# tensorlayer/HyperPose

Hardware: AMD Instinct MI355X
Metric: end-to-end FPS (preproc+DNN+PAF parse) @ 368x432 (higher is better)
Workload: dtype f32; 1 GPU; configs[1]: Lightweight-OpenPose (MobilenetDilated) + PAF parser, batch 8 @ 368x432 per GPU; frames from pinned host memory (one H2D per batch), parser on the network's own maps, humans to the host; key=configs[1]/f32, global_batch=8, parallelism=frame-sharded x1, no steady-state collective, pipes_per_gpu=4, parser_input=the network's own heat-maps

## Files before the change

### hyperpose_amd/csrc/conv32_winograd.hip

```cpp
#include "conv_fp32.hpp"

#include "conv32_epilogue.hpp"
#include "conv_device.hpp"

#include <cstdlib>
#include <vector>

namespace hp {

namespace {

typedef float f32x4 __attribute__((ext_vector_type(4)));

constexpr int WCK = 16;
constexpr int HALO_W = 10;
constexpr int RAW_PB = WCK * 4;
constexpr int VP = 24 * 4;

template <int MW, int NC = 2>
struct wino_geom {
    static constexpr int NT = 64 * MW;
    static constexpr int HALO_H = 8 * NC + 2;
    static constexpr int RAW_Q = HALO_H * HALO_W * 4;
    static constexpr int NQ = (RAW_Q + NT - 1) / NT;
    static constexpr int RAW_BYTES = NQ * NT * 16;
    static constexpr int NI = 4 * NC / MW;
    static_assert(NI >= 1, "a transform item per wavefront");
    static constexpr int TMS = MW / 2;
    static constexpr int SLAB_PITCH = rows_geom<TMS>::PITCH, SLAB_BYTES = 64 * NC * SLAB_PITCH * 4;
    static constexpr int VPOS = 16 * NC * VP, VBUF = 16 * VPOS;
    static constexpr int LDS_BYTES = RAW_BYTES + (VBUF > SLAB_BYTES ? VBUF : SLAB_BYTES);
    static constexpr int PVPOS = 16 * NC * 64, PVBUF = 16 * PVPOS;
    static constexpr int PLDS_BYTES = RAW_BYTES + (2 * PVBUF > SLAB_BYTES ? 2 * PVBUF : SLAB_BYTES);
};

__device__ __forceinline__ long tvw_off(const tview32& t, int b, int y, int x)
{
    return ((long)b * t.img + (long)y * t.wp + x) * t.cs + t.coff;
}

}

template <int MW, bool PIPE, int NC = 2>
__global__ __launch_bounds__(64 * MW, MW == 8 ? 1 : NC == 1 ? 3 : 2) void conv32_winograd_kernel(const conv32_params p, int tiles_x, int tiles_y, int vh)
{
    static_assert(!PIPE || MW == 4, "the pipelined form is the four-wavefront one");
    using G = wino_geom<MW, NC>;
    constexpr int NT = G::NT, NQ = G::NQ, SLAB_PITCH = G::SLAB_PITCH, RAW_Q = G::RAW_Q, VPOS = G::VPOS;
    extern __shared__ __attribute__((aligned(16))) unsigned char lds[];
    unsigned char* const raw = lds;
    unsigned char* const vb = lds + G::RAW_BYTES;

    const int tid = threadIdx.x, lane = tid & 63, wave = tid >> 6;
    const int NG = p.Cout_pad / (16 * MW), ntiles = tiles_x * tiles_y * (vh ? 1 : p.B);
    const int Hin = vh ? (p.B - 1) * vh + p.H : p.H;
    const int bj = blockIdx.x >> 3, by = bj % NG;
    int t = (bj / NG) * 8 + (blockIdx.x & 7);
    if (t >= ntiles)
        return;
    const int bx = t;
    const int tx = t % tiles_x;
    t /= tiles_x;
    const int ty = t % tiles_y, b = t / tiles_y;
    const int y0 = ty * (8 * NC), x0 = tx * 8;
    const int MT = p.Cout_pad / 16, mt = by * MW + wave;
    const int nch = p.Cin / WCK;
    int dbg_i = 0;
#define HP_STAMP()                                                     \
    if (p.dbg && bx == 1 && by == 0 && tid == 0)       \
        p.dbg[dbg_i++] = __builtin_amdgcn_s_memtime();
    HP_STAMP();
    if (p.dbg && bx == 1 && by == 0 && tid == 0)
        p.dbg[119] = __builtin_readcyclecounter(), p.dbg[120] = __builtin_amdgcn_s_memrealtime();

    long goff[NQ];
    bool qok[NQ];
#pragma unroll
    for (int i = 0; i < NQ; ++i) {
        const int q = min(tid + i * NT, RAW_Q - 1);
        const int hp = q >> 2, c4 = q & 3;
        const int hy = hp / HALO_W, hx = hp - hy * HALO_W;
        const int y = y0 - 1 + hy, x = x0 - 1 + hx;
        qok[i] = y <= Hin && x <= p.W;
        goff[i] = tvw_off(p.in, b, min(y, Hin), min(x, p.W)) + c4 * 4;
    }
    f32x4 stage[NQ];
    auto gload = [&](int c) {
#pragma unroll
        for (int i = 0; i < NQ; ++i)
            stage[i] = *reinterpret_cast<const f32x4*>(p.in.p + goff[i] + min(c, nch - 1) * WCK);
    };
    auto to_lds = [&]() {
#pragma unroll
        for (int i = 0; i < NQ; ++i)
            *reinterpret_cast<f32x4*>(raw + (tid + i * NT) * 16) = qok[i] ? stage[i] : f32x4{ 0.f, 0.f, 0.f, 0.f };
    };
    auto transform = [&]() {
#pragma unroll
        for (int k = 0; k < G::NI; ++k) {
            const int item = wave + k * MW, i = NC == 2 ? item >> 1 : item;
            const int quad = lane >> 4, tile = (NC == 2 ? (item & 1) * 16 : 0) + (lane & 15);
            const int ra = i == 0 ? 0 : i == 2 ? 2 : 1, rb = i == 0 ? 2 : i == 1 ? 2 : i == 2 ? 1 : 3;
            const float sg = i == 1 ? 1.f : -1.f;
            const unsigned char* const src = raw + ((2 * (tile >> 2)) * HALO_W + 2 * (tile & 3)) * RAW_PB + quad * 16;
            f32x4 T[4];
#pragma unroll
            for (int j = 0; j < 4; ++j) {
                const f32x4 a = *reinterpret_cast<const f32x4*>(src + (ra * HALO_W + j) * RAW_PB);
                const f32x4 bq = *reinterpret_cast<const f32x4*>(src + (rb * HALO_W + j) * RAW_PB);
                T[j] = a + sg * bq;
            }
            constexpr int PS = PIPE ? G::PVPOS : VPOS;
            unsigned char* const dst = PIPE ? vb + (i * 4) * PS + tile * 64 + ((quad ^ ((4 - (tile >> 2)) & 3)) * 16) : vb + (i * 4) * PS + tile * VP + quad * 16;
            *reinterpret_cast<f32x4*>(dst) = T[0] - T[2];
            *reinterpret_cast<f32x4*>(dst + PS) = T[1] + T[2];
            *reinterpret_cast<f32x4*>(dst + 2 * PS) = T[2] - T[1];
            *reinterpret_cast<f32x4*>(dst + 3 * PS) = T[1] - T[3];
        }
    };
    f32x4 ta[4], tb[4];
    auto transform_piece = [&](int pos, int buf) {
        const int k = pos >> 3, ps = pos & 7;
        if (k >= G::NI)
            return;
        const int item = wave + k * MW, i = NC == 2 ? item >> 1 : item;
        const int quad = lane >> 4, tile = (NC == 2 ? (item & 1) * 16 : 0) + (lane & 15);
        const int ra = i == 0 ? 0 : i == 2 ? 2 : 1, rb = i == 0 ? 2 : i == 1 ? 2 : i == 2 ? 1 : 3;
        const unsigned char* const src = raw + ((2 * (tile >> 2)) * HALO_W + 2 * (tile & 3)) * RAW_PB + quad * 16;
        if (ps < 4) {
            ta[ps] = *reinterpret_cast<const f32x4*>(src + (ra * HALO_W + ps) * RAW_PB);
            tb[ps] = *reinterpret_cast<const f32x4*>(src + (rb * HALO_W + ps) * RAW_PB);
        } else {
            if (ps == 4) {
                const float sg = i == 1 ? 1.f : -1.f;
#pragma unroll
                for (int j = 0; j < 4; ++j)
                    ta[j] = ta[j] + sg * tb[j];
            }
            unsigned char* const dst = vb + buf * G::PVBUF + (i * 4 + (ps - 4)) * G::PVPOS + tile * 64 + ((quad ^ ((4 - (tile >> 2)) & 3)) * 16);
            *reinterpret_cast<f32x4*>(dst) = ps == 4 ? ta[0] - ta[2] : ps == 5 ? ta[1] + ta[2] : ps == 6 ? ta[2] - ta[1] : ta[1] - ta[3];
        }
    };

    const long step_stride = (long)MT * 256;
    const float* const wp = p.w_wino + (long)mt * 256 + lane * 4;
    const int nsteps = nch * 16;
    constexpr int RING = PIPE ? 4 : 8, AHEAD = PIPE ? 3 : 6;
    f32x4 fa[RING];
    auto aload = [&](int slot, int s) { fa[slot] = *reinterpret_cast<const f32x4*>(wp + (long)min(s, nsteps - 1) * step_stride); };

    f32x4 acc[16][NC];
#pragma unroll
    for (int i = 0; i < 16; ++i)
#pragma unroll
        for (int nc = 0; nc < NC; ++nc)
            acc[i][nc] = f32x4{ 0.f, 0.f, 0.f, 0.f };

    const int btile = lane & 15, kq = lane >> 4;
    const unsigned char* const vsrc = PIPE ? vb + btile * 64 + ((kq ^ ((4 - (btile >> 2)) & 3)) * 16) : vb + btile * VP + kq * 16;
    constexpr int BPOS = PIPE ? G::PVPOS : VPOS, BNT = PIPE ? 16 * 64 : 16 * VP;

    gload(0);
#pragma unroll
    for (int a = 0; a < AHEAD; ++a)
        aload(a, a);
    if constexpr (PIPE) {
        to_lds();
        gload(1);
        lds_barrier();
        transform();
    }
    int s = 0;
#pragma unroll 1
    for (int c = 0; c < nch; ++c) {
        if constexpr (PIPE)
            lds_barrier();
        to_lds();
        gload(PIPE ? c + 2 : c + 1);
        lds_barrier();
        HP_STAMP();
        if constexpr (!PIPE) {
            transform();
            lds_barrier();
            HP_STAMP();
        }
        const unsigned char* const vcur = vsrc + (PIPE ? (c & 1) * G::PVBUF : 0);
        f32x4 fb[2][NC];
#pragma unroll
        for (int nc = 0; nc < NC; ++nc)
            fb[0][nc] = *reinterpret_cast<const f32x4*>(vcur + nc * BNT);
#pragma unroll
        for (int pos = 0; pos < 16; ++pos) {
            const int cur = pos & 1, npos = pos + 1 < 16 ? pos + 1 : pos;
#pragma unroll
            for (int nc = 0; nc < NC; ++nc)
                fb[cur ^ 1][nc] = *reinterpret_cast<const f32x4*>(vcur + npos * BPOS + nc * BNT);
            aload((pos + AHEAD) % RING, s + AHEAD);
            const int slot = pos % RING;
#pragma unroll
            for (int e = 0; e < 4; ++e)
#pragma unroll
                for (int nc = 0; nc < NC; ++nc)
                    acc[pos][nc] = __builtin_amdgcn_mfma_f32_16x16x4f32(fa[slot][e], fb[cur][nc][e], acc[pos][nc], 0, 0, 0);
            if constexpr (PIPE)
                transform_piece(pos, (c + 1) & 1);
            __builtin_amdgcn_sched_group_barrier(0x008, 1, 0);
            __builtin_amdgcn_sched_group_barrier(0x100, 1, 0);
            if constexpr (NC == 2) {
                __builtin_amdgcn_sched_group_barrier(0x008, 1, 0);
                __builtin_amdgcn_sched_group_barrier(0x100, 1, 0);
            }
            __builtin_amdgcn_sched_group_barrier(0x008, 1, 0);
            __builtin_amdgcn_sched_group_barrier(0x020, 1, 0);
            __builtin_amdgcn_sched_group_barrier(0x008, NC == 2 ? 5 : 2, 0);
            __builtin_amdgcn_sched_barrier(0);
            ++s;
        }
        HP_STAMP();
    }

    lds_barrier();
    HP_STAMP();
    float* const slab = reinterpret_cast<float*>(vb);
#pragma unroll
    for (int nt = 0; nt < NC; ++nt) {
        f32x4 S[2][4];
#pragma unroll
        for (int j = 0; j < 4; ++j) {
            S[0][j] = acc[j][nt] + acc[4 + j][nt] + acc[8 + j][nt];
            S[1][j] = acc[4 + j][nt] - acc[8 + j][nt] - acc[12 + j][nt];
        }
#pragma unroll
        for (int a = 0; a < 2; ++a) {
            const f32x4 y0v = S[a][0] + S[a][1] + S[a][2], y1v = S[a][1] - S[a][2] - S[a][3];
            *reinterpret_cast<f32x4*>(slab + ((a * 2 + 0) * (16 * NC) + nt * 16 + btile) * SLAB_PITCH + wave * 16 + kq * 4) = y0v;
            *reinterpret_cast<f32x4*>(slab + ((a * 2 + 1) * (16 * NC) + nt * 16 + btile) * SLAB_PITCH + wave * 16 + kq * 4) = y1v;
        }
    }
    HP_STAMP();
    lds_barrier();
    HP_STAMP();
    constexpr int RPW = 64 * NC / MW;
    conv32_drain_rows<G::TMS, RPW>(p, slab + wave * RPW * SLAB_PITCH, lane, by * 16 * MW, [&](int r, bool& ok, long& ooff, long& roff) {
        const int rr = wave * RPW + r, ab = rr / (16 * NC), tile = rr % (16 * NC);
        int oy = y0 + 2 * (tile >> 2) + (ab >> 1), ob = b;
        const int ox = x0 + 2 * (tile & 3) + (ab & 1);
        if (vh)
            ob = oy / vh, oy -= ob * vh;
        ok = oy < p.OH && ox < p.OW && ob < p.B;
        const int oyc = min(oy, p.OH - 1), oxc = min(ox, p.OW - 1), obc = min(ob, p.B - 1);
        ooff = tvw_off(p.out, obc, oyc, oxc);
        roff = p.res.p ? tvw_off(p.res, obc, oyc, oxc) : 0;
    });
    HP_STAMP();
#undef HP_STAMP
    if (p.dbg && bx == 1 && by == 0 && tid == 0)
        p.dbg[121] = __builtin_readcyclecounter(), p.dbg[122] = __builtin_amdgcn_s_memrealtime();
}

bool conv32_winograd_ok(const conv32_params& p)
{
    return p.KH == 3 && p.KW == 3 && p.stride == 1 && p.dil == 1 && p.Cin % WCK == 0 && p.Cout_pad % 64 == 0 && p.OH == p.H && p.OW == p.W && p.pad_t == 1
        && p.pad_l == 1 && !p.out_f32 && p.out.p;
}

int conv32_winograd_tile(const conv32_params& p) { return p.w_wino3 ? conv32_winograd3_tile(p) : 35000000 + 3000 + 4; }

double conv32_winograd_flops(const conv32_params& p)
{
    return 2.0 * 16 * (double)p.B * ((p.OH + 1) / 2) * ((p.OW + 1) / 2) * p.Cout * p.Cin;
}

void conv32_winograd_pack(const float* packed, int cout_pad, int cin, float* out)
{
    static const double G[4][3] = { { 1, 0, 0 }, { .5, .5, .5 }, { .5, -.5, .5 }, { 0, 0, 1 } };
    const int nch = cin / WCK, MT = cout_pad / 16;
    std::vector<double> U((size_t)16 * cout_pad * cin);
    for (int m = 0; m < cout_pad; ++m)
        for (int k = 0; k < cin; ++k) {
            double g[3][3], Gg[4][3];
            for (int t = 0; t < 9; ++t)
                g[t / 3][t % 3] = packed[((size_t)t * cout_pad + m) * cin + k];
            for (int i = 0; i < 4; ++i)
                for (int j = 0; j < 3; ++j)
                    Gg[i][j] = G[i][0] * g[0][j] + G[i][1] * g[1][j] + G[i][2] * g[2][j];
            for (int i = 0; i < 4; ++i)
                for (int j = 0; j < 4; ++j)
                    U[((size_t)(i * 4 + j) * cout_pad + m) * cin + k] = Gg[i][0] * G[j][0] + Gg[i][1] * G[j][1] + Gg[i][2] * G[j][2];
        }
    for (int c = 0; c < nch; ++c)
        for (int pos = 0; pos < 16; ++pos)
            for (int mt = 0; mt < MT; ++mt) {
                float* dst = out + (((size_t)c * 16 + pos) * MT + mt) * 256;
                for (int lane = 0; lane < 64; ++lane)
                    for (int e = 0; e < 4; ++e) {
                        const int m = mt * 16 + (lane & 15), k = c * WCK + (lane >> 4) * 4 + e;
                        dst[lane * 4 + e] = (float)U[((size_t)pos * cout_pad + m) * cin + k];
                    }
            }
}

template <int MW, bool PIPE, int NC = 2>
static hipError_t launch_wino_case(const conv32_params& q, dim3 grid, int tiles_x, int tiles_y, int vh, hipStream_t s)
{
    constexpr int lds = PIPE ? wino_geom<MW, NC>::PLDS_BYTES : wino_geom<MW, NC>::LDS_BYTES;
    static bool granted = false;
    if (lds > 64 * 1024 && !granted) {
        const hipError_t e = hipFuncSetAttribute((const void*)conv32_winograd_kernel<MW, PIPE, NC>, hipFuncAttributeMaxDynamicSharedMemorySize, lds);
        if (e != hipSuccess)
            return e;
        granted = true;
    }
    HP_LAUNCH((conv32_winograd_kernel<MW, PIPE, NC>), grid, dim3(64 * MW), lds, s, q, tiles_x, tiles_y, vh);
    return hipGetLastError();
}

static int winograd_nc(const conv32_params& p, const engine_switches& sw, int blocks_nc2)
{
    const int force = sw.wino_nc;
    if (force == 1 || force == 2)
        return force;
    return p.latency && blocks_nc2 <= 512 ? 1 : 2;
}

static int winograd_tall(const conv32_params& p, const engine_switches& sw)
{
    if (!sw.wino_tall)
        return 0;
    if (p.B < 2 || p.in.wp <= 0 || p.in.img % p.in.wp)
        return 0;
    const int vh = p.in.img / p.in.wp;
    return (vh & 1) == 0 && vh >= p.H + 2 ? vh : 0;
}

hipError_t launch_conv32_winograd(const conv32_params& p, const engine_switches& sw, hipStream_t s)
{
    if (!conv32_winograd_ok(p) || !p.w_wino || p.npix <= 0)
        return hipErrorInvalidValue;
    constexpr int mw = 4;
    const int tiles_x = (p.OW + 7) / 8;
    const int nc = winograd_nc(p, sw, tiles_x * ((p.OH + 15) / 16) * p.B * (p.Cout_pad / 64)), bh = 8 * nc;
    int tiles_y = (p.OH + bh - 1) / bh, vh = winograd_tall(p, sw), images = p.B;
    if (vh) {
        const int tall_y = ((p.B - 1) * vh + p.H + bh - 1) / bh;
        if (tall_y < tiles_y * p.B)
            tiles_y = tall_y, images = 1;
        else
            vh = 0;
    }
    const dim3 grid((tiles_x * tiles_y * images + 7) / 8 * 8 * (p.Cout_pad / (16 * mw)));
    if (nc == 1)
        return launch_wino_case<4, true, 1>(p, grid, tiles_x, tiles_y, vh, s);
    return launch_wino_case<4, true>(p, grid, tiles_x, tiles_y, vh, s);
}

hipError_t conv32_winograd_occupancy(const conv32_params&, int* blocks_per_cu)
{
    return hipOccupancyMaxActiveBlocksPerMultiprocessor(blocks_per_cu, conv32_winograd_kernel<4, true>, 256, wino_geom<4>::PLDS_BYTES);
}

}
```

### hyperpose_amd/csrc/engine.cpp

```cpp
#include "conv_fp32.hpp"
#include "conv_i8.hpp"
#include "conv_kernels.hpp"
#include "hp_common.hpp"

#include <algorithm>
#include <cmath>
#include <map>
#include <memory>
#include <string>
#include <cstdio>
#include <cstdlib>
#include <vector>

namespace {

inline int round_up(int a, int b) { return (a + b - 1) / b * b; }

struct tensor_info {
    bool defined = false;
    bool elided = false;
    bool unwritten = false;
    int H = 0, W = 0, C = 0;
    int cs = 0;
    int P = 0;
// ... 1478 lines not shown
}

int hp_engine::pair_heads()
{
    const bool f32 = is_f32();
    if (!switches.no_pair_heads && !f32) {
        for (size_t k = 0; k + 1 < steps.size(); ++k) {
            step &a = steps[k], &b = steps[k + 1];
            if (a.op != OP_MLPHEAD || b.op != OP_MLPHEAD || a.paired)
                continue;
            const auto &x = a.hp_, &y = b.hp_;
            if (x.in.p != y.in.p || x.in.coff != y.in.coff || x.K1 != y.K1 || x.H != y.H || x.W != y.W || x.pw.Cout > 64 || y.pw.Cout > 64)
                continue;
            a.hp2_ = b.hp_, a.paired = true, a.n_layers += b.n_layers;
            a.flops += b.flops, a.bytes += b.bytes;
            steps.erase(steps.begin() + k + 1);
        }
    }
    return HP_OK;
}

int hp_engine::finish(const hp_engine_desc* d)
{
    HP_REQUIRE(!steps.empty() && steps[0].first, HP_ERR_INVALID, "engine: the first layer must be a CONV reading tensor 0");

    HP_HIP_TRY(hipStreamCreateWithFlags(&stream, hipStreamNonBlocking));
    HP_HIP_TRY(hipEventCreate(&ev0));
    HP_HIP_TRY(hipEventCreate(&ev1));
    HP_HIP_TRY(hipEventCreateWithFlags(&ev_fork, hipEventDisableTiming));
    HP_HIP_TRY(hipEventCreateWithFlags(&ev_join, hipEventDisableTiming));
    if (dtype == HP_DTYPE_I8) {
        i8_scale.assign(layers.size(), 0.f);
        for (size_t i = 0; i < layers.size(); ++i)
            if (i8_eligible((int)i))
                i8_scale[i] = -1.f;
        if (d->int8_scales) {
            HP_TRY(check_int8_scales(d->int8_scales, d->n_layers, true));
            i8_scale.assign(d->int8_scales, d->int8_scales + d->n_layers);
            for (auto& v : i8_scale)
                v = v < 0.f ? -1.f : v;
        }
        HP_TRY(apply_int8_scales());
    }
    return HP_OK;
}


int hp_engine::check_int8_scales(const float* s, int n, bool allow_uncalibrated) const
{
    HP_REQUIRE(s, HP_ERR_INVALID, "int8 scales: null vector");
    HP_REQUIRE(n == (int)layers.size(), HP_ERR_INVALID, "int8 scales: %d values for %zu layers", n, layers.size());
    for (int i = 0; i < n; ++i) {
        HP_REQUIRE(std::isfinite(s[i]), HP_ERR_INVALID, "int8 scales: layer %d: %g is not finite", i, (double)s[i]);
        const bool uncal = allow_uncalibrated && s[i] == -1.f && i8_eligible(i);
        HP_REQUIRE(s[i] >= 0.f || uncal, HP_ERR_INVALID, "int8 scales: layer %d: negative scale %g", i, (double)s[i]);
        HP_REQUIRE(s[i] <= 0.f || i8_eligible(i), HP_ERR_INVALID,
            "int8 scales: layer %d has no int8 kernel (first layer, depthwise, pooling or an uncovered geometry): its scale must be 0", i);
    }
    return HP_OK;
}

int hp_engine::apply_int8_scales()
{
    for (auto& st : steps) {
        if (!st.i8)
            continue;
        const float sa = i8_scale[st.layer];
        const std::vector<float>& s_w = i8_sw[st.layer];
        std::vector<float> dq(st.cp.Cout_pad, 0.f);
        if (sa > 0.f)
            for (size_t c = 0; c < s_w.size(); ++c)
                dq[c] = sa * s_w[c];
        st.q8.inv_a = sa > 0.f ? 1.0f / sa : 0.f;
        HP_HIP_TRY(hipMemcpy(st.i8_dq, dq.data(), dq.size() * sizeof(float), hipMemcpyHostToDevice));
    }
    return HP_OK;
}

int hp_engine::drop_graphs()
{
    HP_HIP_TRY(hipStreamSynchronize(stream));
    if (last.stream)
        HP_HIP_TRY(hipStreamSynchronize((hipStream_t)last.stream));
    if (stream2)
        HP_HIP_TRY(hipStreamSynchronize(stream2));
    for (auto& g : graphs)
        (void)hipGraphExecDestroy(g.second);
    graphs.clear();
    return HP_OK;
}

namespace {
inline hp::tview32 at_frame(hp::tview32 v, int b0)
{
    if (v.p)
        v.p += (long)b0 * v.img * v.cs;
    return v;
}
hp::conv32_params at_frame(hp::conv32_params p, int b0)
{
    p.in = at_frame(p.in, b0), p.out = at_frame(p.out, b0), p.res = at_frame(p.res, b0);
    if (p.out_f32)
        p.out_f32 += (size_t)b0 * p.Cout * p.OH * p.OW;
    return p;
}
hp::dw32_params at_frame(hp::dw32_params p, int b0)
{
    p.in = at_frame(p.in, b0), p.out = at_frame(p.out, b0);
    return p;
}
hp::pool32_params at_frame(hp::pool32_params p, int b0)
{
    p.in = at_frame(p.in, b0), p.out = at_frame(p.out, b0);
    return p;
}

void print_conv32_residency(const unsigned long long* h)
{
    struct blk { unsigned long long t0, t1; unsigned cu; };
    std::vector<blk> bl;
    unsigned long long tmin = ~0ull, tmax = 0;
    for (int b = 0; b < 4096; ++b) {
        const unsigned long long t0 = h[128 + 3 * b], t1 = h[128 + 3 * b + 1], id = h[128 + 3 * b + 2];
        if (!t0 || !t1)
            continue;
        bl.push_back({ t0, t1, (unsigned)(((id >> 32) & 0xf) << 8 | ((id >> 8) & 0xff)) });
        tmin = std::min(tmin, t0), tmax = std::max(tmax, t1);
    }
    if (bl.empty())
        return;
    std::map<unsigned, std::vector<std::pair<unsigned long long, int>>> ev;
    double dsum = 0, dmin = 1e30, dmax = 0;
    for (const auto& b : bl) {
        ev[b.cu].push_back({ b.t0, +1 }), ev[b.cu].push_back({ b.t1, -1 });
        const double d = (b.t1 - b.t0) * 0.01;
        dsum += d, dmin = std::min(dmin, d), dmax = std::max(dmax, d);
    }
    int peak = 0;
    std::map<int, int> blocks_per_cu, peak_hist;
    for (auto& kv : ev) {
        std::sort(kv.second.begin(), kv.second.end());
        int cur = 0, pk = 0;
        for (auto& e2 : kv.second)
            cur += e2.second, pk = std::max(pk, cur);
        peak = std::max(peak, pk), ++peak_hist[pk], ++blocks_per_cu[(int)kv.second.size() / 2];
    }
    fprintf(stderr, "  residency: %zu blocks on %zu CUs in %.2f us (first start -> last end); block duration %.2f .. %.2f us, mean %.2f; peak resident blocks per CU:",
        bl.size(), ev.size(), (tmax - tmin) * 0.01, dmin, dmax, dsum / bl.size());
    for (auto& kv : peak_hist)
        fprintf(stderr, " %d x%d", kv.first, kv.second);
    fprintf(stderr, "; blocks run per CU:");
    for (auto& kv : blocks_per_cu)
        fprintf(stderr, " %d x%d", kv.first, kv.second);
    fprintf(stderr, "; active blocks at 10 %% .. 90 %% of the launch:");
    for (int k = 1; k < 10; ++k) {
        const unsigned long long t = tmin + (tmax - tmin) * k / 10;
        int a = 0;
        for (const auto& b : bl)
            a += b.t0 <= t && t < b.t1;
        fprintf(stderr, " %d", a);
    }
    fprintf(stderr, "; block 9: %.2f us", (h[128 + 3 * 9 + 1] - h[128 + 3 * 9]) * 0.01);
    fprintf(stderr, "; durations (10 bins from min to max):");
    int hist[10] = { 0 };
    for (const auto& b : bl)
        ++hist[std::min(9, (int)(((b.t1 - b.t0) * 0.01 - dmin) / std::max(1e-9, dmax - dmin) * 10))];
    for (int k = 0; k < 10; ++k)
        fprintf(stderr, " %d", hist[k]);
    double xs[16] = { 0 };
    int xn[16] = { 0 };
    for (const auto& b : bl)
        xs[(b.cu >> 8) & 15] += (b.t1 - b.t0) * 0.01, ++xn[(b.cu >> 8) & 15];
    fprintf(stderr, "; mean duration per XCD:");
    for (int k = 0; k < 16; ++k)
        if (xn[k])
            fprintf(stderr, " %.1f", xs[k] / xn[k]);
    double late0 = 1e30, late_d = 0;
    int nlate = 0;
    for (const auto& b : bl)
        if ((b.t0 - tmin) * 0.01 > 5.0)
            late0 = std::min(late0, (b.t0 - tmin) * 0.01), late_d += (b.t1 - b.t0) * 0.01, ++nlate;
    if (nlate)
        fprintf(stderr, "; %d blocks started later than 5 us after the first (earliest at %.1f us), their mean duration %.2f us", nlate, late0, late_d / nlate);
    fprintf(stderr, "\n");
}

struct block_spans {
    int nb = 0;
    unsigned long long t0 = ~0ull, t1 = 0, smax = 0, dmin = ~0ull, dmax = 0, dsum = 0;
    explicit block_spans(const unsigned long long* h)
    {
        for (int i = 0; i < 1024 && h[64 + 2 * i]; ++i, ++nb) {
            const unsigned long long d = h[65 + 2 * i] - h[64 + 2 * i];
            t0 = std::min(t0, h[64 + 2 * i]), t1 = std::max(t1, h[65 + 2 * i]), smax = std::max(smax, h[64 + 2 * i]);
            dmin = std::min(dmin, d), dmax = std::max(dmax, d), dsum += d;
        }
    }
};
}

int hp_engine::print_timeline(const step& st, const hp::conv32_params* q32, hipStream_t s)
{
    enum { NONE, CONV, BNECK, CHAIN, SEP, WINO3, WINO, DIRECT, CONV32 } kind = NONE;
    size_t words = 0;
    if (q32 && st.f32 && st.op == HP_OP_CONV && !st.first && !st.head32 && switches.dbg_direct) {
        kind = st.wino ? (q32->w_wino3 ? WINO3 : WINO) : st.cin_split ? DIRECT : q32->Cin >= switches.dbg_min_cin ? CONV32 : NONE;
        words = kind == WINO ? 128 : kind == CONV32 ? 128 + 3 * 4096 : 64;
    } else if (!st.f32 && st.op == HP_OP_CONV && !st.first && !i8_on(st) && switches.dbg_conv && hp::conv_mfma_tile(st.cp) / 100000 == 52)
        kind = CONV, words = 64;
    else if (st.op == OP_BNECK && switches.dbg_bn)
        kind = BNECK, words = 64 + 2 * 1024;
    else if (st.op == OP_CHAIN && switches.dbg_chain)
        kind = CHAIN, words = 32;
    else if (st.op == OP_SEPCONV && !st.sep_pair && switches.dbg_sep)
        kind = SEP, words = 64 + 2 * 1024 + 64;
    if (kind == NONE)
        return HP_OK;
    hp::dev_buf buf;
    HP_TRY(buf.alloc(words * 8));
    HP_HIP_TRY(hipMemset(buf.p, 0, words * 8));
    unsigned long long* const dbg = buf.as<unsigned long long>();
    hp::conv32_params q = q32 ? *q32 : hp::conv32_params{};
    q.dbg = dbg;
    const bool split = dtype == HP_DTYPE_F32S && !split_off;
    if (kind == CONV) {
        hp::conv_params c = st.cp;
        c.dbg = dbg;
        HP_HIP_TRY(hp::launch_conv_mfma(c, s));
    } else if (kind == BNECK) {
        hp::bneck_params b = st.bn;
        b.ce.dbg = dbg;
        HP_HIP_TRY(hp::launch_bottleneck(b, s));
    } else if (kind == CHAIN) {
        hp::chain_params c = st.ch;
        c.c2.dbg = dbg;
        HP_HIP_TRY(hp::launch_conv_chain(c, s));
    } else if (kind == SEP) {
        hp::sep_params p = st.sp;
        p.pw.dbg = dbg;
        HP_HIP_TRY(hp::launch_sepconv(p, s));
    } else if (kind == WINO3)
        HP_HIP_TRY(hp::launch_conv32_winograd3(q, s));
    else if (kind == WINO)
        HP_HIP_TRY(hp::launch_conv32_winograd(q, switches, s));
    else if (kind == DIRECT)
        HP_HIP_TRY(hp::launch_conv32_direct(q, split, s));
    else
        HP_HIP_TRY(hp::launch_conv32(q, switches, s));
    HP_HIP_TRY(hipStreamSynchronize(s));
    std::vector<unsigned long long> hv(words);
    const unsigned long long* h = hv.data();
    HP_HIP_TRY(hipMemcpy(hv.data(), dbg, words * 8, hipMemcpyDeviceToHost));
    auto deltas = [h](int from, int to) {
        for (int i = from; i < to && h[i]; ++i)
            fprintf(stderr, " %llu", h[i] - h[i - 1]);
    };
    switch (kind) {
    case CONV:
        fprintf(stderr, "conv layer %d %d->%d tile %d consumer:", st.layer, st.cp.Cin, st.cp.Cout, hp::conv_mfma_tile(st.cp));
        deltas(1, 32);
        fprintf(stderr, " | producer (from consumer start %lld):", (long long)(h[32] - h[0]));
        deltas(33, 64);
        fprintf(stderr, "\n");
        break;
    case BNECK: {
        fprintf(stderr, "bottleneck layer %d variant %d timeline:", st.layer, hp::bottleneck_variant(st.bn));
        deltas(1, 60);
        const block_spans b(h);
        if (b.nb)
            fprintf(stderr, "\n  first %d blocks: %.2f us from first start to last end; block duration %.2f .. %.2f us, mean %.2f", b.nb, (b.t1 - b.t0) * 0.01,
                b.dmin * 0.01, b.dmax * 0.01, b.dsum * 0.01 / b.nb);
        fprintf(stderr, "\n");
        break;
    }
    case CHAIN:
        fprintf(stderr, "chain layer %d variant %d timeline:", st.layer, hp::conv_chain_variant(st.ch));
        deltas(1, 32);
        fprintf(stderr, "\n");
        break;
    case SEP:
        fprintf(stderr, "sep layer %d C=%d timeline:", st.layer, st.sp.C);
        deltas(1, 40);
        if (h[41])
            fprintf(stderr, " | total-to-epi0 %llu pass1 %llu epi1 %llu | total %llu", h[41] - h[0], h[42] - h[41], h[43] - h[42], h[43] - h[0]);
        fprintf(stderr, "\n");
        if (h[2112]) {
            fprintf(stderr, "  wavefront 4 of block 1:");
            for (int i = 1; i < 40 && h[2112 + i]; ++i)
                fprintf(stderr, " %llu", h[2112 + i] - h[2112 + i - 1]);
            fprintf(stderr, "\n");
        }
        if (h[64]) {
            const block_spans b(h);
            fprintf(stderr, "  %d blocks: first start -> last end %.2f us, starts spread over %.2f us, block duration %.2f .. %.2f us\n", b.nb,
                (b.t1 - b.t0) * 0.01, (b.smax - b.t0) * 0.01, b.dmin * 0.01, b.dmax * 0.01);
        }
        break;
    case WINO3:
        fprintf(stderr, "winograd3 layer %d %d->%d cycles [start | chunk 0 transformed | per chunk: patch stored, multiplied | output transformed | stored]:", st.layer, q.Cin, q.Cout);
        deltas(1, 60);
        fprintf(stderr, "\n");
        break;
    case WINO: {
        fprintf(stderr, "winograd layer %d %d->%d tile %d cycles [start | staged, transformed, multiplied per chunk | stored]:", st.layer, q.Cin, q.Cout,
            hp::conv32_winograd_tile(q));
        deltas(1, 119);
        int occ = 0;
        (void)hp::conv32_winograd_occupancy(q, &occ);
        fprintf(stderr, " | s_memtime ticks %llu in %llu ticks of the 100 MHz clock; blocks per CU %d\n", h[121] - h[119], h[122] - h[120], occ);
        break;
    }
    case DIRECT:
        fprintf(stderr, "direct layer %d %dx%d %d->%d tile %d cycles [start | staged, multiplied per chunk | stored]:", st.layer, q.KH, q.KW, q.Cin, q.Cout,
            hp::conv32_direct_tile(q, split));
        deltas(1, 64);
        fprintf(stderr, "\n");
        break;
    default:
        fprintf(stderr, "conv32 layer %d %dx%d %d->%d tile %d cycles [start | staged | per 8 K-steps | stored]:", st.layer, q.KH, q.KW, q.Cin, q.Cout, hp::conv32_tile(q, switches));
        deltas(1, 128);
        fprintf(stderr, "\n");
        print_conv32_residency(h);
        break;
    }
    return HP_OK;
}

int hp_engine::run_step(step& st, const uint8_t* u8, const float* f32, int n, hipStream_t s, int b0)
{
    if (st.f32) {
        const size_t in_off = (size_t)b0 * in_h * in_w * 3;
        hp::conv32_params moved;
        hp::conv32_params& cp = b0 ? (moved = at_frame(st.cp32, b0)) : st.cp32;
        if (st.first) {
            hp::first_conv32_params p = st.fp32;
            p.out = at_frame(p.out, b0);
            p.in_u8 = u8 ? u8 + in_off : nullptr, p.in_f32 = f32 ? f32 + in_off : nullptr, p.B = n;
            if (!b0)
                st.fp32 = p;
            HP_HIP_TRY(hp::launch_first_conv32(p, switches, s));
        } else if (st.op == HP_OP_CONV) {
            cp.B = n, cp.npix = n * cp.OH * cp.OW;
            if (st.head32) {
                HP_HIP_TRY(hp::launch_conv32_head(cp, st.hh, s));
            } else if (st.wino) {
                cp.latency = parts > 1;
                if (cp.w_wino3)
                    HP_HIP_TRY(hp::launch_conv32_winograd3(cp, s));
                else
                    HP_HIP_TRY(hp::launch_conv32_winograd(cp, switches, s));
            } else if (st.cin_split) {
                hp::conv32_params q = cp;
                q.Cin = st.cin_split;
                HP_HIP_TRY(hp::launch_conv32_direct(q, dtype == HP_DTYPE_F32S && !split_off, s));
                return print_timeline(st, &q, s);
            } else
                HP_HIP_TRY(hp::launch_conv32(cp, switches, s));
            return print_timeline(st, &cp, s);
        } else if (st.op == HP_OP_DWCONV) {
            hp::dw32_params p = b0 ? at_frame(st.dp32, b0) : st.dp32;
            p.B = n;
            if (!b0)
                st.dp32.B = n;
            HP_HIP_TRY(hp::launch_dwconv32(p, switches, s));
        } else {
            hp::pool32_params p = b0 ? at_frame(st.pp32, b0) : st.pp32;
            p.B = n;
            if (!b0)
                st.pp32.B = n;
            HP_HIP_TRY(st.op == HP_OP_UPSAMPLE ? hp::launch_upsample32(p, s) : hp::launch_maxpool32(p, s));
        }
        return HP_OK;
    }
    if (st.first) {
        st.fp.in_u8 = u8, st.fp.in_f32 = f32, st.fp.B = n;
        HP_HIP_TRY(hp::launch_first_conv(st.fp, s));
    } else if (st.op == HP_OP_CONV && i8_on(st)) {
        st.cp.B = n, st.cp.npix = n * st.cp.OH * st.cp.OW;
        st.q8.c = st.cp;
        HP_HIP_TRY(hp::launch_conv_i8(st.q8, s));
    } else if (st.op == HP_OP_CONV) {
        st.cp.B = n, st.cp.npix = n * st.cp.OH * st.cp.OW;
        HP_HIP_TRY(hp::launch_conv_mfma(st.cp, s));
    } else if (st.op == OP_BNECK) {
        st.bn.c3.B = st.bn.ce.B = st.bn.cr.B = n;
        HP_HIP_TRY(hp::launch_bottleneck(st.bn, s));
    } else if (st.op == OP_CHAIN) {
        st.ch.c0.B = st.ch.c1.B = st.ch.c2.B = n;
        HP_HIP_TRY(hp::launch_conv_chain(st.ch, s));
    } else if (st.op == OP_SEPCONV) {
        st.sp.B = n, st.sp.pw.B = n, st.sp.pw.npix = n * st.sp.OH * st.sp.OW;
        if (st.sep_pair) {
            st.sp2.B = n, st.sp2.pw.B = n, st.sp2.pw.npix = n * st.sp2.OH * st.sp2.OW;
            HP_HIP_TRY(hp::launch_seppair(hp::seppair_params{ st.sp, st.sp2 }, s));
        } else
            HP_HIP_TRY(hp::launch_sepconv(st.sp, s));
    } else if (st.op == OP_MLPHEAD) {
        st.hp_.B = n, st.hp_.pw.B = n;
        if (st.paired) {
            st.hp2_.B = n, st.hp2_.pw.B = n;
            HP_HIP_TRY(hp::launch_mlp_head_pair(st.hp_, st.hp2_, s));
        } else
            HP_HIP_TRY(hp::launch_mlp_head(st.hp_, s));
    } else if (st.op == HP_OP_DWCONV) {
        st.dp.B = n;
        HP_HIP_TRY(hp::launch_dwconv3x3(st.dp, s));
    } else if (st.op == HP_OP_UPSAMPLE) {
        st.pp.B = n;
        HP_HIP_TRY(hp::launch_upsample(st.pp, s));
    } else {
        st.pp.B = n;
        HP_HIP_TRY(hp::launch_maxpool(st.pp, s));
    }
    return print_timeline(st, nullptr, s);
}

int hp_engine::enqueue_range(const uint8_t* u8, const float* f32, int b0, int n, hipStream_t s)
{
    for (size_t i = 0; i < steps.size(); ++i) {
        step& st = steps[i];
        if (st.f32 && st.head32 && i + 1 < steps.size() && steps[i + 1].f32 && steps[i + 1].head32) {
            hp::conv32_params a = at_frame(st.cp32, b0), b = at_frame(steps[i + 1].cp32, b0);
            for (hp::conv32_params* q : { &a, &b })
                q->B = n, q->npix = n * q->OH * q->OW;
            if (hp::conv32_head_pair_ok(a, b, switches)) {
                HP_HIP_TRY(hp::launch_conv32_head_pair(a, st.hh, b, steps[i + 1].hh, s));
                ++i;
                continue;
            }
        }
        HP_TRY(run_step(st, u8, f32, n, s, b0));
    }
    for (auto& o : outputs)
        if (o.fused_layer < 0) {
            const tensor_info& ti = *tensors[o.tensor];
            float* const dst = o.buf->as<float>() + (size_t)b0 * o.out_c() * o.x.out_h * o.x.out_w;
            if (is_f32())
                HP_HIP_TRY(hp::launch_output_transform32(at_frame(ti.view32(o.coff), b0), n, o.H, o.W, o.x, dst, s));
            else
                HP_HIP_TRY(hp::launch_output_transform(ti.view(o.coff), n, o.H, o.W, o.x, dst, s));
        }
    return HP_OK;
}

int hp_engine::step_tile(const step& st) const
{
    if (st.op == OP_SEPCONV)
        return 4000000 + (st.sep_pair ? 20 : hp::sepconv_variant(st.sp));
    if (st.op == OP_MLPHEAD)
        return 6000000 + st.hp_.K1;
    if (st.op == OP_CHAIN)
        return 7000000 + hp::conv_chain_variant(st.ch);
    if (st.op == OP_BNECK)
        return 9000000 + hp::bottleneck_variant(st.bn);
    if (st.op != HP_OP_CONV || st.first)
        return 0;
    if (!st.f32)
        return i8_on(st) ? hp::conv_i8_tile(st.cp) : hp::conv_mfma_tile(st.cp);
    return st.head32 ? hp::conv32_head_tile(st.hh.HID, st.cp32.Cout)
        : st.wino    ? hp::conv32_winograd_tile(st.cp32)
        : st.cin_split ? hp::conv32_direct_tile(st.cp32, dtype == HP_DTYPE_F32S && !split_off)
                     : hp::conv32_tile(st.cp32, switches);
}

int hp_engine::stage_profile_input()
{
    const size_t need = (size_t)max_batch * in_h * in_w * 3 * sizeof(float);
    if (in_stage.bytes < need)
        HP_TRY(in_stage.alloc(need));
    return HP_OK;
}

int hp_engine::enqueue(const uint8_t* u8, const float* f32, int n, hipStream_t s, const void* host_src, size_t frame_bytes)
{
    unsigned char* const dev_in = u8 ? (unsigned char*)u8 : (unsigned char*)f32;
    auto h2d = [&](int b0, int cnt, hipStream_t st) -> int {
        if (host_src)
            HP_HIP_TRY(hipMemcpyAsync(dev_in + (size_t)b0 * frame_bytes, (const unsigned char*)host_src + (size_t)b0 * frame_bytes, (size_t)cnt * frame_bytes, hipMemcpyHostToDevice, st));
        return HP_OK;
    };
    if (parts < 2 || !halves_ok() || n < 2) {
        HP_TRY(h2d(0, n, s));
        return enqueue_range(u8, f32, 0, n, s);
    }
    const int n0 = (n + 1) / 2;
    HP_HIP_TRY(hipEventRecord(ev_fork, s));
    HP_HIP_TRY(hipStreamWaitEvent(stream2, ev_fork, 0));
    HP_TRY(h2d(0, n0, s));
    HP_TRY(h2d(n0, n - n0, stream2));
    HP_TRY(enqueue_range(u8, f32, 0, n0, s));
    HP_TRY(enqueue_range(u8, f32, n0, n - n0, stream2));
    HP_HIP_TRY(hipEventRecord(ev_join, stream2));
    HP_HIP_TRY(hipStreamWaitEvent(s, ev_join, 0));
    return HP_OK;
}

hp::engine_switches hp::read_engine_switches()
{
    auto on = [](const char* name) { return getenv(name) != nullptr; };
    auto num = [](const char* name, int unset) { const char* v = getenv(name); return v ? atoi(v) : unset; };
    engine_switches w;
    w.no_fuse = on("HP_NO_FUSE"), w.no_fuse_head = num("HP_NO_FUSE_HEAD", 0) != 0, w.no_splitk = on("HP_NO_SPLITK");
    w.no_chain = on("HP_NO_CHAIN"), w.no_bneck = on("HP_NO_BNECK"), w.no_seppair = on("HP_NO_SEPPAIR"), w.no_pair_heads = on("HP_NO_PAIR_HEADS");
    w.fuse32 = on("HP_FUSE32"), w.no_fuse32 = on("HP_NO_FUSE32"), w.no_head32 = on("HP_NO_HEAD32"), w.no_arena = on("HP_NO_ARENA");
    w.no_winograd32 = on("HP_NO_WINOGRAD32"), w.wino_f33 = num("HP_WINO_F33", 0) == 1, w.wino_tall = num("HP_WINO_TALL", 1) != 0;
    w.wino_nc = num("HP_WINO_NC", 0), w.head_pair32 = num("HP_HEAD_PAIR", 1) != 0;
    w.c32_wk = num("HP_C32_WK", -1), w.c32_bn160 = num("HP_C32_BN160", -1), w.dw32_px = num("HP_DW32_PX", 0);
    w.lane_epilogue = num("HP_LANE_EPILOGUE", 0), w.first_conv_verify = on("HP_FIRST_CONV_VERIFY");
    w.dbg_conv = on("HP_CONV_DBG"), w.dbg_bn = on("HP_BN_DBG"), w.dbg_chain = on("HP_CHAIN_DBG"), w.dbg_sep = on("HP_SEP_DBG");
    w.dbg_direct = on("HP_DIRECT_DBG"), w.dbg_min_cin = num("HP_DIRECT_DBG_MINCIN", 256);
    return w;
}

extern "C" {

int hp_engine_create(hp_engine** out, const hp_engine_desc* desc)
{
    HP_REQUIRE(out && desc, HP_ERR_INVALID, "hp_engine_create: null argument");
    std::unique_ptr<hp_engine> e(new hp_engine());
    e->switches = hp::read_engine_switches();
    try {
        HP_TRY(e->build(desc));
    } catch (const std::exception& ex) {
        HP_REQUIRE(false, HP_ERR_INVALID, "hp_engine_create: %s", ex.what());
    }
    *out = e.release();
    return HP_OK;
}

namespace {
constexpr char ENGINE_MAGIC[8] = { 'H', 'P', 'E', 'N', 'G', '0', '0', '3' };
struct engine_file_header {
    char magic[8];
    int32_t layer_size, output_size;
    int32_t in_w, in_h, max_batch, flip_rb;
    double factor;
    float mean[3], inv_std[3];
    int32_t n_layers, n_outputs;
    uint64_t n_weights;
    int32_t dtype;
    int32_t n_scales;
};
}

int hp_engine_save(const hp_engine* e, const char* path)
{
    HP_REQUIRE(e && path, HP_ERR_INVALID, "hp_engine_save: null argument");
    FILE* f = fopen(path, "wb");
    HP_REQUIRE(f, HP_ERR_INVALID, "hp_engine_save: cannot open %s for writing", path);
    engine_file_header h{};
    memcpy(h.magic, ENGINE_MAGIC, 8);
    h.layer_size = (int32_t)sizeof(hp_layer), h.output_size = (int32_t)sizeof(hp_output_desc);
    h.in_w = e->in_w, h.in_h = e->in_h, h.max_batch = e->max_batch, h.flip_rb = e->flip_rb, h.factor = e->factor;
    for (int c = 0; c < 3; ++c)
        h.mean[c] = e->mean[c], h.inv_std[c] = e->inv_std[c];
    h.n_layers = (int32_t)e->layers.size(), h.n_outputs = (int32_t)e->out_descs.size(), h.n_weights = e->weights_blob.size();
    h.dtype = e->dtype;
    h.n_scales = (int32_t)e->i8_scale.size();
    bool ok = fwrite(&h, sizeof(h), 1, f) == 1;
    ok = ok && fwrite(e->layers.data(), sizeof(hp_layer), e->layers.size(), f) == e->layers.size();
    ok = ok && fwrite(e->out_descs.data(), sizeof(hp_output_desc), e->out_descs.size(), f) == e->out_descs.size();
    ok = ok && fwrite(e->weights_blob.data(), sizeof(float), e->weights_blob.size(), f) == e->weights_blob.size();
    ok = ok && fwrite(e->i8_scale.data(), sizeof(float), e->i8_scale.size(), f) == e->i8_scale.size();
    ok = (fclose(f) == 0) && ok;
    HP_REQUIRE(ok, HP_ERR_INVALID, "hp_engine_save: short write to %s", path);
    return HP_OK;
}

int hp_engine_load(hp_engine** out, const char* path, int max_batch)
{
    HP_REQUIRE(out && path, HP_ERR_INVALID, "hp_engine_load: null argument");
    FILE* f = fopen(path, "rb");
    HP_REQUIRE(f, HP_ERR_INVALID, "hp_engine_load: cannot open %s", path);
    engine_file_header h{};
    std::vector<hp_layer> layers;
    std::vector<hp_output_desc> outs;
    std::vector<float> w, scales;
    constexpr size_t HDR_001 = offsetof(engine_file_header, dtype);
    bool ok = fread(&h, HDR_001, 1, f) == 1;
    if (ok && memcmp(h.magic, "HPENG001", 8) == 0)
        memcpy(h.magic, ENGINE_MAGIC, 8), h.dtype = HP_DTYPE_F16, h.n_scales = 0;
    else {
        ok = ok && fread(reinterpret_cast<char*>(&h) + HDR_001, sizeof(h) - HDR_001, 1, f) == 1;
        if (ok && memcmp(h.magic, "HPENG002", 8) == 0)
            memcpy(h.magic, ENGINE_MAGIC, 8), ok = h.n_scales == 0 && h.dtype != HP_DTYPE_I8;
    }
    ok = ok && memcmp(h.magic, ENGINE_MAGIC, 8) == 0 && h.layer_size == (int32_t)sizeof(hp_layer)
        && h.output_size == (int32_t)sizeof(hp_output_desc) && h.n_layers > 0 && h.n_layers < (1 << 20) && h.n_outputs > 0
        && h.n_outputs < 4096 && h.n_weights < ((uint64_t)1 << 34)
        && (h.dtype == HP_DTYPE_F16 || h.dtype == HP_DTYPE_F32 || h.dtype == HP_DTYPE_F32S || h.dtype == HP_DTYPE_I8)
        && h.n_scales == (h.dtype == HP_DTYPE_I8 ? h.n_layers : 0);
    if (ok) {
        const long at = ftell(f);
        ok = fseek(f, 0, SEEK_END) == 0;
        const long size = ftell(f);
        ok = ok && fseek(f, at, SEEK_SET) == 0
            && (uint64_t)size == (uint64_t)at + (uint64_t)h.n_layers * sizeof(hp_layer) + (uint64_t)h.n_outputs * sizeof(hp_output_desc) + h.n_weights * sizeof(float)
                    + (uint64_t)h.n_scales * sizeof(float);
    }
    if (ok) {
        layers.resize(h.n_layers), outs.resize(h.n_outputs), w.resize(h.n_weights), scales.resize(h.n_scales);
        ok = fread(layers.data(), sizeof(hp_layer), layers.size(), f) == layers.size()
            && fread(outs.data(), sizeof(hp_output_desc), outs.size(), f) == outs.size() && fread(w.data(), sizeof(float), w.size(), f) == w.size()
            && fread(scales.data(), sizeof(float), scales.size(), f) == scales.size();
    }
    fclose(f);
    HP_REQUIRE(ok, HP_ERR_INVALID, "hp_engine_load: %s is not an engine file written by this library version", path);
// ... 468 lines not shown
```

Baseline: 5260 frames/s.

## Pack winograd tile rows across images and hoist epilogue loads before output transform

Adds a row-packed tiling mode for the winograd conv in which tile rows of consecutive images are concatenated, so blocks no longer leave partial tiles at each image's bottom edge. The input patch grows by one row so it can span an image boundary. The pipelined main loop is restructured so staging of the next patch follows the multiply. The generic drain helper is replaced by an inline epilogue that issues residual, bias and slope loads before the output transform so their latency overlaps it. The cost is more index logic and a larger raw LDS patch.

```diff
diff --git a/hyperpose_amd/csrc/conv32_winograd.hip b/hyperpose_amd/csrc/conv32_winograd.hip
--- a/hyperpose_amd/csrc/conv32_winograd.hip
+++ b/hyperpose_amd/csrc/conv32_winograd.hip
@@ -11,6 +11,8 @@
 namespace {
 
 typedef float f32x4 __attribute__((ext_vector_type(4)));
+typedef __attribute__((address_space(1))) float gfloat;
+typedef __attribute__((address_space(1))) f32x4 gf32x4;
 
 constexpr int WCK = 16;
 constexpr int HALO_W = 10;
@@ -20,8 +22,10 @@
 template <int MW, int NC = 2>
 struct wino_geom {
     static constexpr int NT = 64 * MW;
+    static constexpr int TB = 4 * NC;
     static constexpr int HALO_H = 8 * NC + 2;
-    static constexpr int RAW_Q = HALO_H * HALO_W * 4;
+    static constexpr int PATCH_H = HALO_H + 1;
+    static constexpr int RAW_Q = PATCH_H * HALO_W * 4;
     static constexpr int NQ = (RAW_Q + NT - 1) / NT;
     static constexpr int RAW_BYTES = NQ * NT * 16;
     static constexpr int NI = 4 * NC / MW;
@@ -42,17 +46,17 @@
 }
 
 template <int MW, bool PIPE, int NC = 2>
-__global__ __launch_bounds__(64 * MW, MW == 8 ? 1 : NC == 1 ? 3 : 2) void conv32_winograd_kernel(const conv32_params p, int tiles_x, int tiles_y, int vh)
+__global__ __launch_bounds__(64 * MW, MW == 8 ? 1 : NC == 1 ? 3 : 2) void conv32_winograd_kernel(const conv32_params p, int tiles_x, int tiles_y, int vh, int T)
 {
     static_assert(!PIPE || MW == 4, "the pipelined form is the four-wavefront one");
     using G = wino_geom<MW, NC>;
-    constexpr int NT = G::NT, NQ = G::NQ, SLAB_PITCH = G::SLAB_PITCH, RAW_Q = G::RAW_Q, VPOS = G::VPOS;
+    constexpr int NT = G::NT, NQ = G::NQ, SLAB_PITCH = G::SLAB_PITCH, VPOS = G::VPOS;
     extern __shared__ __attribute__((aligned(16))) unsigned char lds[];
     unsigned char* const raw = lds;
     unsigned char* const vb = lds + G::RAW_BYTES;
 
     const int tid = threadIdx.x, lane = tid & 63, wave = tid >> 6;
-    const int NG = p.Cout_pad / (16 * MW), ntiles = tiles_x * tiles_y * (vh ? 1 : p.B);
+    const int NG = p.Cout_pad / (16 * MW), ntiles = tiles_x * tiles_y * (vh || T ? 1 : p.B);
     const int Hin = vh ? (p.B - 1) * vh + p.H : p.H;
     const int bj = blockIdx.x >> 3, by = bj % NG;
     int t = (bj / NG) * 8 + (blockIdx.x & 7);
@@ -73,16 +77,25 @@
     if (p.dbg && bx == 1 && by == 0 && tid == 0)
         p.dbg[119] = __builtin_readcyclecounter(), p.dbg[120] = __builtin_amdgcn_s_memrealtime();
 
+    int kb = G::TB, sh = 0, img0 = b, ly0 = y0 - 1, l0 = 0;
+    if (T) {
+        const int r0 = ty * G::TB;
+        img0 = r0 / T, l0 = r0 - img0 * T, ly0 = 2 * l0 - 1;
+        kb = min(T - l0, G::TB), sh = kb < G::TB && !(p.H & 1);
+    }
+    const int Hlim = T ? p.H : Hin, ylow = kb < G::TB ? 2 * kb + 1 + sh : G::PATCH_H;
+    const int nvalid = (G::HALO_H + sh) * HALO_W * 4;
     long goff[NQ];
     bool qok[NQ];
 #pragma unroll
     for (int i = 0; i < NQ; ++i) {
-        const int q = min(tid + i * NT, RAW_Q - 1);
+        const int q = min(tid + i * NT, nvalid - 1);
         const int hp = q >> 2, c4 = q & 3;
         const int hy = hp / HALO_W, hx = hp - hy * HALO_W;
-        const int y = y0 - 1 + hy, x = x0 - 1 + hx;
-        qok[i] = y <= Hin && x <= p.W;
-        goff[i] = tvw_off(p.in, b, min(y, Hin), min(x, p.W)) + c4 * 4;
+        const bool below = hy >= ylow;
+        const int bi = below ? img0 + 1 : img0, y = below ? hy - ylow : ly0 + hy, x = x0 - 1 + hx;
+        qok[i] = y <= Hlim && x <= p.W && bi < p.B;
+        goff[i] = tvw_off(p.in, min(bi, p.B - 1), min(y, Hlim), min(x, p.W)) + c4 * 4;
     }
     f32x4 stage[NQ];
     auto gload = [&](int c) {
@@ -94,6 +107,10 @@
 #pragma unroll
         for (int i = 0; i < NQ; ++i)
             *reinterpret_cast<f32x4*>(raw + (tid + i * NT) * 16) = qok[i] ? stage[i] : f32x4{ 0.f, 0.f, 0.f, 0.f };
+    };
+    auto tile_src = [&](int tile, int quad) {
+        const int tr = tile >> 2;
+        return raw + ((2 * tr + (tr >= kb ? sh : 0)) * HALO_W + 2 * (tile & 3)) * RAW_PB + quad * 16;
     };
     auto transform = [&]() {
 #pragma unroll
@@ -102,20 +119,20 @@
             const int quad = lane >> 4, tile = (NC == 2 ? (item & 1) * 16 : 0) + (lane & 15);
             const int ra = i == 0 ? 0 : i == 2 ? 2 : 1, rb = i == 0 ? 2 : i == 1 ? 2 : i == 2 ? 1 : 3;
             const float sg = i == 1 ? 1.f : -1.f;
-            const unsigned char* const src = raw + ((2 * (tile >> 2)) * HALO_W + 2 * (tile & 3)) * RAW_PB + quad * 16;
-            f32x4 T[4];
+            const unsigned char* const src = tile_src(tile, quad);
+            f32x4 Td[4];
 #pragma unroll
             for (int j = 0; j < 4; ++j) {
                 const f32x4 a = *reinterpret_cast<const f32x4*>(src + (ra * HALO_W + j) * RAW_PB);
                 const f32x4 bq = *reinterpret_cast<const f32x4*>(src + (rb * HALO_W + j) * RAW_PB);
-                T[j] = a + sg * bq;
+                Td[j] = a + sg * bq;
             }
             constexpr int PS = PIPE ? G::PVPOS : VPOS;
             unsigned char* const dst = PIPE ? vb + (i * 4) * PS + tile * 64 + ((quad ^ ((4 - (tile >> 2)) & 3)) * 16) : vb + (i * 4) * PS + tile * VP + quad * 16;
-            *reinterpret_cast<f32x4*>(dst) = T[0] - T[2];
-            *reinterpret_cast<f32x4*>(dst + PS) = T[1] + T[2];
-            *reinterpret_cast<f32x4*>(dst + 2 * PS) = T[2] - T[1];
-            *reinterpret_cast<f32x4*>(dst + 3 * PS) = T[1] - T[3];
+            *reinterpret_cast<f32x4*>(dst) = Td[0] - Td[2];
+            *reinterpret_cast<f32x4*>(dst + PS) = Td[1] + Td[2];
+            *reinterpret_cast<f32x4*>(dst + 2 * PS) = Td[2] - Td[1];
+            *reinterpret_cast<f32x4*>(dst + 3 * PS) = Td[1] - Td[3];
         }
     };
     f32x4 ta[4], tb[4];
@@ -126,7 +143,7 @@
         const int item = wave + k * MW, i = NC == 2 ? item >> 1 : item;
         const int quad = lane >> 4, tile = (NC == 2 ? (item & 1) * 16 : 0) + (lane & 15);
         const int ra = i == 0 ? 0 : i == 2 ? 2 : 1, rb = i == 0 ? 2 : i == 1 ? 2 : i == 2 ? 1 : 3;
-        const unsigned char* const src = raw + ((2 * (tile >> 2)) * HALO_W + 2 * (tile & 3)) * RAW_PB + quad * 16;
+        const unsigned char* const src = tile_src(tile, quad);
         if (ps < 4) {
             ta[ps] = *reinterpret_cast<const f32x4*>(src + (ra * HALO_W + ps) * RAW_PB);
             tb[ps] = *reinterpret_cast<const f32x4*>(src + (rb * HALO_W + ps) * RAW_PB);
@@ -161,25 +178,33 @@
     constexpr int BPOS = PIPE ? G::PVPOS : VPOS, BNT = PIPE ? 16 * 64 : 16 * VP;
 
     gload(0);
-#pragma unroll
-    for (int a = 0; a < AHEAD; ++a)
-        aload(a, a);
     if constexpr (PIPE) {
+#pragma unroll
+        for (int a = 0; a < AHEAD; ++a)
+            aload(a, a);
         to_lds();
         gload(1);
         lds_barrier();
+        HP_STAMP();
         transform();
+        lds_barrier();
+        to_lds();
+        gload(2);
+        lds_barrier();
+        HP_STAMP();
+    } else {
+#pragma unroll
+        for (int a = 0; a < AHEAD; ++a)
+            aload(a, a);
     }
     int s = 0;
 #pragma unroll 1
     for (int c = 0; c < nch; ++c) {
-        if constexpr (PIPE)
+        if constexpr (!PIPE) {
+            to_lds();
+            gload(c + 1);
             lds_barrier();
-        to_lds();
-        gload(PIPE ? c + 2 : c + 1);
-        lds_barrier();
-        HP_STAMP();
-        if constexpr (!PIPE) {
+            HP_STAMP();
             transform();
             lds_barrier();
             HP_STAMP();
@@ -217,8 +242,68 @@
             ++s;
         }
         HP_STAMP();
-    }
-
+        if constexpr (PIPE) {
+            if (c + 1 < nch) {
+                lds_barrier();
+                to_lds();
+                gload(c + 3);
+                lds_barrier();
+                HP_STAMP();
+            }
+        }
+    }
+
+    int tid_o = tid;
+    asm volatile("" : "+v"(tid_o));
+    const int lane_o = tid_o & 63, btile_o = lane_o & 15, kq_o = lane_o >> 4;
+    using R = rows_geom<G::TMS>;
+    constexpr int RPW = 64 * NC / MW, NPASS = RPW / R::RPP;
+    static_assert(RPW % R::RPP == 0, "slab rows per pass");
+    const int dc4 = lane_o % R::LPR, dm = by * 16 * MW + dc4 * 4;
+    const bool dany = dm < p.Cout, quads = (p.Cout & 3) == 0;
+    const bool out_vec = quads && ((p.out.coff | p.out.cs) & 3) == 0, res_vec = quads && ((p.res.coff | p.res.cs) & 3) == 0;
+    const int dmc = dany ? dm : 0;
+    int dpix[NPASS], rpix[NPASS];
+    bool dok[NPASS];
+#pragma unroll
+    for (int k = 0; k < NPASS; ++k) {
+        const int rr = wave * RPW + k * R::RPP + lane_o / R::LPR, ab = rr / (16 * NC), tile = rr % (16 * NC), tr = tile >> 2;
+        const int ox = x0 + 2 * (tile & 3) + (ab & 1);
+        int oy, ob;
+        if (T)
+            ob = tr >= kb ? img0 + 1 : img0, oy = 2 * (tr >= kb ? tr - kb : l0 + tr) + (ab >> 1);
+        else {
+            oy = y0 + 2 * tr + (ab >> 1);
+            ob = vh ? oy / vh : b, oy -= vh ? ob * vh : 0;
+        }
+        dok[k] = oy < p.OH && ox < p.OW && ob < p.B && dany;
+        const int oyc = min(oy, p.OH - 1), oxc = min(ox, p.OW - 1), obc = min(ob, p.B - 1);
+        dpix[k] = (obc * p.out.img + oyc * p.out.wp) + oxc;
+        rpix[k] = (obc * p.res.img + oyc * p.res.wp) + oxc;
+    }
+    f32x4 dres[NPASS];
+#pragma unroll
+    for (int k = 0; k < NPASS; ++k)
+        dres[k] = f32x4{ 0.f, 0.f, 0.f, 0.f };
+    const gfloat* const gres = (const gfloat*)p.res.p;
+    gfloat* const gout = (gfloat*)p.out.p;
+    if (gres) {
+        if (res_vec) {
+#pragma unroll
+            for (int k = 0; k < NPASS; ++k)
+                dres[k] = *reinterpret_cast<const gf32x4*>(gres + ((long)rpix[k] * p.res.cs + p.res.coff + dmc));
+        } else {
+#pragma unroll
+            for (int k = 0; k < NPASS; ++k)
+#pragma unroll
+                for (int e = 0; e < 4; ++e)
+                    dres[k][e] = gres[(long)rpix[k] * p.res.cs + p.res.coff + min(dm + e, p.Cout - 1)];
+        }
+    }
+    const f32x4 dbs = *(const gf32x4*)(p.bias + dm);
+    f32x4 dsl = { p.act_slope, p.act_slope, p.act_slope, p.act_slope };
+    if (p.alpha)
+        dsl = *(const gf32x4*)(p.alpha + dm);
     lds_barrier();
     HP_STAMP();
     float* const slab = reinterpret_cast<float*>(vb);
@@ -233,25 +318,46 @@
 #pragma unroll
         for (int a = 0; a < 2; ++a) {
             const f32x4 y0v = S[a][0] + S[a][1] + S[a][2], y1v = S[a][1] - S[a][2] - S[a][3];
-            *reinterpret_cast<f32x4*>(slab + ((a * 2 + 0) * (16 * NC) + nt * 16 + btile) * SLAB_PITCH + wave * 16 + kq * 4) = y0v;
-            *reinterpret_cast<f32x4*>(slab + ((a * 2 + 1) * (16 * NC) + nt * 16 + btile) * SLAB_PITCH + wave * 16 + kq * 4) = y1v;
+            *reinterpret_cast<f32x4*>(slab + ((a * 2 + 0) * (16 * NC) + nt * 16 + btile_o) * SLAB_PITCH + wave * 16 + kq_o * 4) = y0v;
+            *reinterpret_cast<f32x4*>(slab + ((a * 2 + 1) * (16 * NC) + nt * 16 + btile_o) * SLAB_PITCH + wave * 16 + kq_o * 4) = y1v;
         }
     }
     HP_STAMP();
     lds_barrier();
     HP_STAMP();
-    constexpr int RPW = 64 * NC / MW;
-    conv32_drain_rows<G::TMS, RPW>(p, slab + wave * RPW * SLAB_PITCH, lane, by * 16 * MW, [&](int r, bool& ok, long& ooff, long& roff) {
-        const int rr = wave * RPW + r, ab = rr / (16 * NC), tile = rr % (16 * NC);
-        int oy = y0 + 2 * (tile >> 2) + (ab >> 1), ob = b;
-        const int ox = x0 + 2 * (tile & 3) + (ab & 1);
-        if (vh)
-            ob = oy / vh, oy -= ob * vh;
-        ok = oy < p.OH && ox < p.OW && ob < p.B;
-        const int oyc = min(oy, p.OH - 1), oxc = min(ox, p.OW - 1), obc = min(ob, p.B - 1);
-        ooff = tvw_off(p.out, obc, oyc, oxc);
-        roff = p.res.p ? tvw_off(p.res, obc, oyc, oxc) : 0;
-    });
+    const float* const wslab = slab + (wave * RPW + lane_o / R::LPR) * SLAB_PITCH + dc4 * 4;
+    f32x4 dv[NPASS];
+#pragma unroll
+    for (int k = 0; k < NPASS; ++k)
+        dv[k] = *reinterpret_cast<const f32x4*>(wslab + k * R::RPP * SLAB_PITCH);
+#pragma unroll
+    for (int k = 0; k < NPASS; ++k) {
+        f32x4 o;
+#pragma unroll
+        for (int e = 0; e < 4; ++e) {
+            float x = dv[k][e] + dbs[e];
+            if (p.res.p && p.res_before_act)
+                x += dres[k][e];
+            x = x > 0.f ? fminf(x, p.act_hi) : x * dsl[e];
+            if (p.res.p && !p.res_before_act)
+                x += dres[k][e];
+            o[e] = x;
+        }
+        dv[k] = o;
+    }
+    if (out_vec) {
+#pragma unroll
+        for (int k = 0; k < NPASS; ++k)
+            if (dok[k])
+                *reinterpret_cast<gf32x4*>(gout + ((long)dpix[k] * p.out.cs + p.out.coff + dm)) = dv[k];
+    } else {
+#pragma unroll
+        for (int k = 0; k < NPASS; ++k)
+#pragma unroll
+            for (int e = 0; e < 4; ++e)
+                if (dok[k] && dm + e < p.Cout)
+                    gout[(long)dpix[k] * p.out.cs + p.out.coff + dm + e] = dv[k][e];
+    }
     HP_STAMP();
 #undef HP_STAMP
     if (p.dbg && bx == 1 && by == 0 && tid == 0)
@@ -301,7 +407,7 @@
 }
 
 template <int MW, bool PIPE, int NC = 2>
-static hipError_t launch_wino_case(const conv32_params& q, dim3 grid, int tiles_x, int tiles_y, int vh, hipStream_t s)
+static hipError_t launch_wino_case(const conv32_params& q, dim3 grid, int tiles_x, int tiles_y, int vh, int rows, hipStream_t s)
 {
     constexpr int lds = PIPE ? wino_geom<MW, NC>::PLDS_BYTES : wino_geom<MW, NC>::LDS_BYTES;
     static bool granted = false;
@@ -311,7 +417,7 @@
             return e;
         granted = true;
     }
-    HP_LAUNCH((conv32_winograd_kernel<MW, PIPE, NC>), grid, dim3(64 * MW), lds, s, q, tiles_x, tiles_y, vh);
+    HP_LAUNCH((conv32_winograd_kernel<MW, PIPE, NC>), grid, dim3(64 * MW), lds, s, q, tiles_x, tiles_y, vh, rows);
     return hipGetLastError();
 }
 
@@ -340,8 +446,11 @@
     constexpr int mw = 4;
     const int tiles_x = (p.OW + 7) / 8;
     const int nc = winograd_nc(p, sw, tiles_x * ((p.OH + 15) / 16) * p.B * (p.Cout_pad / 64)), bh = 8 * nc;
-    int tiles_y = (p.OH + bh - 1) / bh, vh = winograd_tall(p, sw), images = p.B;
-    if (vh) {
+    int tiles_y = (p.OH + bh - 1) / bh, vh = winograd_tall(p, sw), images = p.B, rows = 0;
+    const int T = (p.OH + 1) / 2, rows_y = (p.B * T + 4 * nc - 1) / (4 * nc);
+    if (sw.wino_tall && p.B > 1 && T >= 4 * nc && rows_y < tiles_y * p.B)
+        tiles_y = rows_y, images = 1, rows = T, vh = 0;
+    else if (vh) {
         const int tall_y = ((p.B - 1) * vh + p.H + bh - 1) / bh;
         if (tall_y < tiles_y * p.B)
             tiles_y = tall_y, images = 1;
@@ -350,8 +459,8 @@
     }
     const dim3 grid((tiles_x * tiles_y * images + 7) / 8 * 8 * (p.Cout_pad / (16 * mw)));
     if (nc == 1)
-        return launch_wino_case<4, true, 1>(p, grid, tiles_x, tiles_y, vh, s);
-    return launch_wino_case<4, true>(p, grid, tiles_x, tiles_y, vh, s);
+        return launch_wino_case<4, true, 1>(p, grid, tiles_x, tiles_y, vh, rows, s);
+    return launch_wino_case<4, true>(p, grid, tiles_x, tiles_y, vh, rows, s);
 }
 
 hipError_t conv32_winograd_occupancy(const conv32_params&, int* blocks_per_cu)
diff --git a/hyperpose_amd/csrc/engine.cpp b/hyperpose_amd/csrc/engine.cpp
--- a/hyperpose_amd/csrc/engine.cpp
+++ b/hyperpose_amd/csrc/engine.cpp
@@ -1804,7 +1804,7 @@
         fprintf(stderr, "\n");
         break;
     case WINO: {
-        fprintf(stderr, "winograd layer %d %d->%d tile %d cycles [start | staged, transformed, multiplied per chunk | stored]:", st.layer, q.Cin, q.Cout,
+        fprintf(stderr, "winograd layer %d %d->%d tile %d cycles [chunk 0 staged | transformed, chunk 1 stored | per chunk: multiplied, next patch stored | epilogue requests | output transform | slab complete | stored]:", st.layer, q.Cin, q.Cout,
             hp::conv32_winograd_tile(q));
         deltas(1, 119);
         int occ = 0;
```

After: 5373 frames/s, median of 6. 1.02x the previous value.
